# Alexander-H-Liu/End-to-end-ASR-Pytorch

Hardware: AMD Instinct MI355X
Metric: audio frames/sec training (LAS+CTC, LibriSpeech 80-mel) (higher is better)
Workload: dtype f32; 1 GPU; cfg3: {"B": 32, "T": 1600, "D": 80, "V": 5000, "L": 64}; global_batch=32, parallelism=dp1

## Files before the change

end-to-end-asr-pytorch_amd/_lib.py:

```python
import ctypes
import os

_HERE = os.path.dirname(os.path.abspath(__file__))
LIB_PATH = os.path.join(_HERE, "csrc", "libasrk.so")

c_int, c_i64, c_f32, c_vp, c_sz = (ctypes.c_int, ctypes.c_int64, ctypes.c_float, ctypes.c_void_p,
                                   ctypes.c_size_t)
c_f64 = ctypes.c_double

SIGNATURES = {
    "asrk_version": (c_int, []),
    "asrk_strerror": (ctypes.c_char_p, [c_int]),
    "asrk_init": (c_int, [c_int]),
    "asrk_profile_enable": (None, [c_int]),
    "asrk_profile_families": (None, [ctypes.c_uint]),
    "asrk_profile_reset": (None, []),
    "asrk_profile_get": (c_int, [c_int, ctypes.POINTER(ctypes.c_double), ctypes.POINTER(c_i64)]),
    "asrk_profile_get_work": (c_int, [c_int, ctypes.POINTER(ctypes.c_double)]),
    "asrk_gemm_f32": (c_int, [c_int, c_int, c_int, c_int, c_int, c_f32, c_vp, c_int, c_vp, c_int,
                              c_f32, c_vp, c_int, c_vp, c_vp, c_int, c_int, c_vp, c_sz, c_vp]),
    "asrk_gemm_ws_bytes": (c_sz, [c_int, c_int, c_int, c_int]),
    "asrk_gemm_takes_split": (c_int, [c_int, c_int, c_int, c_int]),
    "asrk_gemm_plan_info": (c_int, [c_int, c_int, c_int, c_int, c_int, c_int, c_int, c_int, c_int, c_f32, c_int, c_int,
                                    c_int, c_vp]),
    "asrk_split_panel_bytes": (ctypes.c_size_t, [c_int, c_int, c_int]),
    "asrk_split_panel_f32": (c_int, [c_vp, c_int, c_int, c_int, c_int, c_vp, c_int, c_vp]),
    "asrk_gemm_panels_f32": (c_int, [c_int, c_int, c_int, c_f32, c_vp, c_int, c_int, c_int, c_int,
                                     c_vp, c_int, c_int, c_int, c_int, c_f32, c_vp, c_int, c_vp, c_vp, c_int, c_vp]),
    "asrk_gemm_panels_splitk_ws_bytes": (c_sz, [c_int, c_int, c_int]),
    "asrk_gemm_panels_splitk_f32": (c_int, [c_int, c_int, c_int, c_f32, c_vp, c_int, c_int, c_int, c_int,
                                            c_vp, c_int, c_int, c_int, c_int, c_f32, c_vp, c_int, c_vp, c_vp, c_int,
                                            c_vp, c_sz, c_int, c_vp]),
    "asrk_copy3d_f32": (c_int, [c_vp, c_vp, c_int, c_int, c_int, c_i64, c_i64, c_i64, c_i64, c_int,
                                c_vp]),
    "asrk_colsum_f32": (c_int, [c_vp, c_int, c_int, c_int, c_vp, c_int, c_vp]),
    "asrk_tanh_fwd_f32": (c_int, [c_vp, c_vp, c_i64, c_vp]),
    "asrk_tanh_bwd_f32": (c_int, [c_vp, c_vp, c_vp, c_i64, c_vp]),
    "asrk_log_softmax_fwd_f32": (c_int, [c_vp, c_vp, c_int, c_int, c_int, c_vp]),
    "asrk_log_softmax_bwd_f32": (c_int, [c_vp, c_vp, c_vp, c_int, c_int, c_int, c_vp]),
    "asrk_cross_entropy_fwd_f32": (c_int, [c_vp, c_int, c_int, c_int, c_vp, c_int, c_vp, c_vp, c_vp]),
    "asrk_cross_entropy_bwd_f32": (c_int, [c_vp, c_int, c_int, c_int, c_vp, c_int, c_vp, c_vp, c_vp,
                                           c_vp]),
    "asrk_cross_entropy_ls_fwd_f32": (c_int, [c_vp, c_int, c_int, c_int, c_vp, c_int, c_vp, c_vp, c_vp, c_vp]),
    "asrk_cross_entropy_ls_bwd_f32": (c_int, [c_vp, c_int, c_int, c_int, c_vp, c_int, c_f32, c_vp, c_vp, c_vp,
                                              c_vp]),
    "asrk_ctc_prefix_score_f32": (c_int, [c_vp, c_vp, c_vp, c_vp, c_vp, c_vp, c_vp, c_int, c_int, c_int,
                                          c_int, c_int, c_int, c_f32, c_vp]),
# ... 221 lines not shown
```

end-to-end-asr-pytorch_amd/csrc/gemm_split.hip:

```cpp
#include "common.h"
#include "knobs.h"
#include <algorithm>
#include <climits>

extern "C" int asrk_cu_count_(void);

namespace {

typedef __bf16 bf16x8 __attribute__((ext_vector_type(8)));

constexpr int PIECE = 1024;

struct SplitGemmArgs {
    const unsigned char *Ap, *Bp;
    float *C;
    const float *bias, *bias2;
    int M, N, ldc;
    int KC;
    size_t rb_stride_a, rb_stride_b;
    int nk;
    int tiles_m, tiles_n;
    float alpha, beta;
    int slices, ldw;
    float *ws;
};

__device__ __forceinline__ void split8(const float (&v)[8], u32x4 (&w)[3]) {
    unsigned h[3][8];
#pragma unroll
    for (int e = 0; e < 8; ++e) {
        const float a = v[e];
        const __bf16 b0 = (__bf16)a;
        const float r1 = a - (float)b0;
        const __bf16 b1 = (__bf16)r1;
        const float r2 = r1 - (float)b1;
        const __bf16 b2 = (__bf16)r2;
        h[0][e] = __builtin_bit_cast(unsigned short, b0);
        h[1][e] = __builtin_bit_cast(unsigned short, b1);
        h[2][e] = __builtin_bit_cast(unsigned short, b2);
// ... 109 lines not shown
    const int kt0 = SK ? (int)((long)slice * p.nk / p.slices) : 0;
    const int nk = SK ? (int)((long)(slice + 1) * p.nk / p.slices) - kt0 : p.nk;
    const int q8 = ntiles >> 3, r8 = ntiles & 7, xcd = bid & 7, loc = bid >> 3;
    const int tile = (xcd < r8 ? xcd * (q8 + 1) : r8 * (q8 + 1) + (xcd - r8) * q8) + loc;
    constexpr int BAND = 8;
    const int band = tile / (BAND * p.tiles_m);
    const int band_w = min(BAND, p.tiles_n - band * BAND);
    const int in_band = tile - band * BAND * p.tiles_m;
    const int tm = in_band / band_w, tn = band * BAND + in_band % band_w;

    const bool loader = !SPEC || wave >= NCW, worker = !SPEC || wave < NCW;
    const int wr = worker ? wave >> 1 : 0, wc = wave & 1;
    const int ltm = tm, ltn = tn;
    const int r0 = (SPEC ? wave - NCW : wave) * RPD;
    const unsigned char *gsrc[RPD];
#pragma unroll
    for (int q = 0; q < RPD; ++q) {
        const int r = r0 + q;
        gsrc[q] = (r < WM ? p.Ap + (size_t)(ltm * WM + r) * p.rb_stride_a
                          : p.Bp + (size_t)(ltn * 2 + r - WM) * p.rb_stride_b);
        if (SK) gsrc[q] += (size_t)kt0 * REGION;
    }
    const unsigned voff = lane * 16;
    unsigned char *ldst = lds + r0 * REGION;
    static_assert((NC * NPL) % 4 == 0, "a region is issued as runs of four pieces");
    auto issue = [&](int kt, int stage) {
        unsigned char *l = ldst + stage * STAGE;
#pragma unroll
        for (int q = 0; q < RPD; ++q) {
            const unsigned char *g = gsrc[q] + (size_t)kt * REGION;
#pragma unroll
            for (int j = 0; j < NC * NPL; j += 4) glds16_run<4>(g + j * PIECE, voff, l + q * REGION + j * PIECE);
        }
    };

    f32x16 acc[2][2];
#pragma unroll
    for (int i = 0; i < 2; ++i)
#pragma unroll
        for (int j = 0; j < 2; ++j)
#pragma unroll
            for (int r = 0; r < 16; ++r) acc[i][j][r] = 0.f;

    const int frag_off = ((lane >> 5) * NPL) * PIECE + (lane & 31) * 16;
    const unsigned char *abase = lds + wr * REGION + frag_off;
// ... 184 lines not shown
    const int wave = __builtin_amdgcn_readfirstlane(tid >> 6);
    const int ntiles = p.tiles_m * p.tiles_n, bid = blockIdx.x;
    const int q8 = ntiles >> 3, r8 = ntiles & 7, xcd = bid & 7, loc = bid >> 3;
    const int tile = (xcd < r8 ? xcd * (q8 + 1) : r8 * (q8 + 1) + (xcd - r8) * q8) + loc;
    const int band = tile / (BAND * p.tiles_m);
    const int band_w = min(BAND, p.tiles_n - band * BAND);
    const int in_band = tile - band * BAND * p.tiles_m;
    const int tm = in_band / band_w, tn = band * BAND + in_band % band_w;
    const int nk = p.nk;

    if (wave >= 4) {
        const int d = wave - 4, first = d * LPT;
        constexpr int NRUN = LPT / 3;
        static_assert(NRUN * 3 == LPT, "runs of three pieces");
        const unsigned char *run_g[NRUN];
#pragma unroll
        for (int k = 0; k < NRUN; ++k) {
            const int idx = first + 3 * k, r = idx / (NC * NPL), j = idx - r * (NC * NPL);
            run_g[k] = (r < 2 ? p.Ap + (size_t)(tm * 2 + r) * p.rb_stride_a
                              : p.Bp + (size_t)min(tn * 4 + r - 2, rb_b - 1) * p.rb_stride_b) + j * PIECE;
        }
        const unsigned voff = lane * 16;
        unsigned char *ldst = lds + first * PIECE;
        auto issue = [&](int kt, int stage) {
            unsigned char *l = ldst + stage * STAGE;
            const size_t gk = (size_t)kt * REGION;
#pragma unroll
            for (int k = 0; k < NRUN; ++k) glds16_run<3>(run_g[k] + gk, voff, l + 3 * k * PIECE);
        };
#pragma unroll
        for (int s = 0; s < NST; ++s)
            if (s < nk) issue(s, s);
        {
            const int later = min(NST - 2, nk - 2);
            if (later >= 2) wait_vm<2 * LPT>();
            else if (later == 1) wait_vm<LPT>();
            else wait_vm<0>();
        }
        __builtin_amdgcn_s_barrier();
        int stage = 0;
        for (int kt = 0; kt < nk; ++kt) {
            const int later = min(NST - 2, nk - 2 - kt);
            if (later >= 2) wait_vm<2 * LPT>();
// ... 165 lines not shown
    const int slice = SK ? blockIdx.x / ntiles : 0, bid = SK ? blockIdx.x - slice * ntiles : blockIdx.x;
    const int kt0 = SK ? (int)((long)slice * p.nk / p.slices) : 0;
    const int nk = SK ? (int)((long)(slice + 1) * p.nk / p.slices) - kt0 : p.nk;
    const int q8 = ntiles >> 3, r8 = ntiles & 7, xcd = bid & 7, loc = bid >> 3;
    const int tile = (xcd < r8 ? xcd * (q8 + 1) : r8 * (q8 + 1) + (xcd - r8) * q8) + loc;
    constexpr int BAND = 8;
    const int band = tile / (BAND * p.tiles_m);
    const int band_w = min(BAND, p.tiles_n - band * BAND);
    const int in_band = tile - band * BAND * p.tiles_m;
    const int tm = in_band / band_w, tn = band * BAND + in_band % band_w;

    const bool worker = wave < 4;
    const int wr = worker ? wave >> 1 : 0, wc = wave & 1;
    const int r0 = worker ? 0 : wave - 4;
    const unsigned char *gsrc = (r0 < 2 ? p.Ap + (size_t)(tm * 2 + r0) * p.rb_stride_a
                                        : p.Bp + (size_t)(tn * 2 + r0 - 2) * p.rb_stride_b) + (size_t)kt0 * REGION;
    const unsigned voff = lane * 16;
    unsigned char *ldst = lds + r0 * REGION;
    auto issue = [&](int kt, int stage) {
        const unsigned char *g = gsrc + (size_t)kt * REGION;
        unsigned char *l = ldst + stage * STAGE;
#pragma unroll
        for (int j = 0; j < LPT; j += 4) glds16_run<4>(g + j * PIECE, voff, l + j * PIECE);
    };

    f32x4 acc[4][4];
#pragma unroll
    for (int i = 0; i < 4; ++i)
#pragma unroll
        for (int j = 0; j < 4; ++j)
#pragma unroll
            for (int r = 0; r < 4; ++r) acc[i][j][r] = 0.f;
    const int frag_off = ((lane >> 4) * NPL) * PIECE + (lane & 15) * 16;
    const unsigned char *abase = lds + wr * REGION + frag_off;
    const unsigned char *bbase = lds + (2 + wc) * REGION + frag_off;
// ... 114 lines not shown
    static_assert(LPT * NDW == NRG * NC * NPL && NRUN * 3 == LPT, "36 pieces per stage, runs of three");
    const int tid = threadIdx.x, lane = tid & 63;
    const int wave = __builtin_amdgcn_readfirstlane(tid >> 6);
    const int ntiles = p.tiles_m * p.tiles_n, bid = blockIdx.x;
    const int q8 = ntiles >> 3, r8 = ntiles & 7, xcd = bid & 7, loc = bid >> 3;
    const int tile = (xcd < r8 ? xcd * (q8 + 1) : r8 * (q8 + 1) + (xcd - r8) * q8) + loc;
    const int band = tile / (BAND * p.tiles_m);
    const int band_w = min(BAND, p.tiles_n - band * BAND);
    const int in_band = tile - band * BAND * p.tiles_m;
    const int tm = in_band / band_w, tn = band * BAND + in_band % band_w;
    const int ns = p.nk >> 1;

    const bool worker = wave < 4;
    const int first = (worker ? 0 : wave - 4) * LPT;
    const unsigned char *run_g[NRUN];
#pragma unroll
    for (int k = 0; k < NRUN; ++k) {
        const int idx = first + 3 * k, r = idx / (NC * NPL), j = idx - r * (NC * NPL);
        run_g[k] = (r < 2 ? p.Ap + (size_t)(tm * 2 + r) * p.rb_stride_a
                          : p.Bp + (size_t)min(tn * 4 + r - 2, rb_b - 1) * p.rb_stride_b) + j * PIECE;
    }
    const unsigned voff = lane * 16;
    unsigned char *ldst = lds + first * PIECE;
    auto issue_pair = [&](int s, int slot) {
#pragma unroll
        for (int h = 0; h < 2; ++h) {
            unsigned char *l = ldst + slot * PAIR + h * STAGE;
            const size_t gk = (size_t)(2 * s + h) * REGION;
#pragma unroll
            for (int k = 0; k < NRUN; ++k) glds16_run<3>(run_g[k] + gk, voff, l + 3 * k * PIECE);
        }
    };

    const int wr = worker ? wave >> 1 : 0, wc = wave & 1;
    f32x4 acc0[4][4], acc1[4][4];
#pragma unroll
    for (int i = 0; i < 4; ++i)
#pragma unroll
        for (int j = 0; j < 4; ++j)
#pragma unroll
            for (int r = 0; r < 4; ++r) acc0[i][j][r] = acc1[i][j][r] = 0.f;
    const int frag_off = (lane >> 5) * STAGE + (((lane >> 4) & 1) * NPL) * PIECE + (lane & 15) * 16;
    const unsigned char *abase = lds + wr * REGION + frag_off;
    const unsigned char *bbase = lds + (2 + wc * 2) * REGION + frag_off;
    bf16x8 fa0[2][4], fa1[4], fa2[4], fb0[4], fb1[4], fb2[4];
// ... 161 lines not shown
        else hipLaunchKernelGGL((split_panel_kernel<false>), grid, dim3(256), 0, s, src, ld, rows, K, dstp, g.KC, g.rb, g.rb_stride);
    }
    asrk_prof_end_(PROF_SPLIT, s);
    ASRK_LAUNCH_CHECK();
    return ASRK_OK;
}

int auto_slices(int M, int N, int nk) {
    if (N >= 512) return 1;
    const int ncu = asrk_cu_count_() > 0 ? asrk_cu_count_() : 256;
    const long tiles = (long)asrk_div_up(M, 128) * asrk_div_up(N, 128);
    const long want = (ncu + tiles - 1) / tiles;
    return (int)std::max(1L, std::min(want, (long)(nk / 64)));
}

int run_panel_gemm(int M, int N, int nk, float alpha, const unsigned char *Ap, size_t stride_a,
                   const unsigned char *Bp, size_t stride_b, float beta, float *C, int ldc, const float *bias,
                   const float *bias2, hipStream_t s, int slices = 1, float *ws = nullptr) {
    const AsrkKnobs &kn = asrk_knobs_();
    SplitGemmArgs a;
    a.Ap = Ap; a.Bp = Bp; a.C = C; a.bias = bias; a.bias2 = bias2;
    a.M = M; a.N = N; a.ldc = ldc; a.KC = 0; a.nk = nk; a.rb_stride_a = stride_a; a.rb_stride_b = stride_b;
    a.tiles_m = asrk_div_up(M, 128); a.tiles_n = asrk_div_up(N, 128);
    a.alpha = alpha; a.beta = beta;
    a.slices = std::min(slices, nk); a.ldw = (N + 3) & ~3; a.ws = ws;
    const bool m16 = kn.is_set(kn.split_mfma) ? kn.split_mfma == 16 : nk >= SPLIT_MFMA16_MIN_NK;
    const bool m16_sk = kn.is_set(kn.split_mfma) && kn.split_mfma == 16;
    const bool m16_128 = m16, m16_w256 = m16;
    if (a.slices > 1) return m16_sk ? launch_split_gemm_m16<true>(a, s) : launch_split_gemm<4, 3, true, 2, true>(a, s);
    const int w256 = kn.get(kn.split_w256, 1);
    if (w256 && N >= 512) {
        const int tm = asrk_div_up(M, 128), tn = asrk_div_up(N, 256);
        const int ncu = asrk_cu_count_() > 0 ? asrk_cu_count_() : 256;
        if (w256 == 2 || (long)tm * tn >= 2L * ncu) {
            SplitGemmArgs b = a;
// ... 61 lines not shown
                                    void *stream) {
    if (!src || !panel || rows <= 0 || K <= 0 || ld < (trans ? rows : K) || flags != 0) return ASRK_EINVAL;
    if ((reinterpret_cast<uintptr_t>(panel) & 15) != 0) return ASRK_EINVAL;
    asrk_prof_begin_(PROF_GEMM, (hipStream_t)stream);
    const int rc = run_split(src, ld, rows, K, trans != 0, reinterpret_cast<unsigned char *>(panel),
                             panel_geom(rows, K, true), (hipStream_t)stream);
    asrk_prof_end_(PROF_GEMM, (hipStream_t)stream);
    return rc;
}

namespace {
struct PanelRange {
    const unsigned char *Ap, *Bp;
    size_t stride_a, stride_b;
    int nk;
};
int panel_range(int M, int N, int K, const void *A_panel, int a_rows, int a_K, int a_row0, int a_k0,
                const void *B_panel, int b_rows, int b_K, int b_row0, int b_k0, const float *C, int ldc, int flags,
                PanelRange &r) {
    if (M <= 0 || N <= 0 || K <= 0 || !A_panel || !B_panel || !C || ldc < N || flags != 0) return ASRK_EINVAL;
    if (a_row0 < 0 || b_row0 < 0 || a_k0 < 0 || b_k0 < 0 || a_row0 % 128 || b_row0 % 128 || a_k0 % 8 || b_k0 % 8)
        return ASRK_EINVAL;
    if (a_row0 + M > a_rows || b_row0 + N > b_rows || a_k0 + K > a_K || b_k0 + K > b_K) return ASRK_EINVAL;
    if (K % 32 != 0 && a_k0 + K != a_K && b_k0 + K != b_K) return ASRK_ESHAPE;
    const PanelGeom ga = panel_geom(a_rows, a_K, true), gb = panel_geom(b_rows, b_K, true);
    r.nk = asrk_div_up(K, 32);
    if (a_k0 / 8 + r.nk * SPLIT_NC > ga.KC || b_k0 / 8 + r.nk * SPLIT_NC > gb.KC) return ASRK_ESHAPE;
    const unsigned char *A0 = reinterpret_cast<const unsigned char *>(A_panel);
    const unsigned char *B0 = reinterpret_cast<const unsigned char *>(B_panel);
    r.Ap = A0 + (size_t)(a_row0 / 64) * ga.rb_stride + (size_t)(a_k0 / 8) * NPL * PIECE;
    r.Bp = B0 + (size_t)(b_row0 / 64) * gb.rb_stride + (size_t)(b_k0 / 8) * NPL * PIECE;
    r.stride_a = ga.rb_stride; r.stride_b = gb.rb_stride;
    return ASRK_OK;
}
}
// ... 28 lines not shown
    if (splitk < 0 || !ws || (reinterpret_cast<uintptr_t>(ws) & 15) != 0) return ASRK_EINVAL;
    PanelRange r;
    const int rc0 = panel_range(M, N, K, A_panel, a_rows, a_K, a_row0, a_k0, B_panel, b_rows, b_K, b_row0, b_k0, C, ldc,
                                flags, r);
    if (rc0 != ASRK_OK) return rc0;
    const int slices = splitk > 0 ? splitk : auto_slices(M, N, r.nk);
    if (ws_bytes < asrk_gemm_panels_splitk_ws_bytes(M, N, slices)) return ASRK_EWORKSPACE;
    hipStream_t s = (hipStream_t)stream;
    asrk_prof_work_(PROF_GEMM, 2.0 * (double)M * (double)N * (double)K);
    asrk_prof_begin_(PROF_GEMM, s);
    const int rc = run_panel_gemm(M, N, r.nk, alpha, r.Ap, r.stride_a, r.Bp, r.stride_b, beta, C, ldc, bias, bias2, s,
                                  slices, reinterpret_cast<float *>(ws));
    asrk_prof_end_(PROF_GEMM, s);
    return rc;
}
```

end-to-end-asr-pytorch_amd/ops.py:

```python
import collections
import contextlib
import ctypes

import numpy as np
import torch
from torch.autograd import Function

from . import _lib

_ws_cache = {}


def _L():
    return _lib.load()


def _require_gpu(t):
    if not t.is_cuda:
        raise _lib.AsrkError("asrk ops need tensors on the MI355X (got %s); the product path has no "
                             "CPU fallback" % t.device)


def _p(t):
    return ctypes.c_void_p(t.data_ptr()) if t is not None else ctypes.c_void_p(0)
# ... 149 lines not shown


def join_deferred():
    for dev, ev in list(_defer["pending"].items()):
        torch.cuda.current_stream(dev).wait_event(ev)
    _defer["pending"].clear()


def deferred_stream(device):
    dev = torch.device(device)
    if dev.index is None:
        dev = torch.device(dev.type, torch.cuda.current_device())
    return _defer["side"].get(dev) if dev in _defer["pending"] else None


def _end_of_backward():
    _defer["cb_armed"] = False
    join_deferred()
    rel, _defer["release"] = _defer["release"], []
    for pnl in rel:
        pnl.release()


def _can_defer(*weights):
    return _defer["enabled"] and all(w is None or (w.is_leaf and w.grad is None) for w in weights)


_BG_FORCED = _os.environ.get("ASRK_SIDE_BG")
_BG_HINT = int(_BG_FORCED) if _BG_FORCED is not None else 0


_gemm_phase_hooks = []
# ... 53 lines not shown
        if self.hint:
            _gemm_state["lds_hint"] = self.hint
        return self

    def keep(self, *outs):
        for t in outs:
            if t is not None:
                t.record_stream(self.main)

    def __exit__(self, *exc):
        _gemm_state["lds_hint"] = self.prev_hint
        self.ctx.__exit__(*exc)
        done = torch.cuda.Event()
        done.record(self.side)
        _defer["pending"][self.device] = done
        if not _defer["cb_armed"]:
            try:
                torch.autograd.Variable._execution_engine.queue_callback(_end_of_backward)
                _defer["cb_armed"] = True
            except RuntimeError:
                join_deferred()
        return False


_grad_dest = {"fn": None}


def set_grad_destination(fn):
    _grad_dest["fn"] = fn


def grad_out(weight, shape, device):
    fn = _grad_dest["fn"]
    if fn is not None and weight is not None:
        t = fn(weight, tuple(shape))
        if t is not None:
# ... 34 lines not shown
        avail = src.untyped_storage().nbytes() // src.element_size() - src.storage_offset()
        if ld < (rows if trans else K) or avail < need:
            raise _lib.AsrkError("split panel: source too small for {}x{} (trans={}) with ld {}".format(
                rows, K, trans, ld))
        self.rows, self.K = rows, K
        self.flags = 0
        self.buf = torch.empty((L.asrk_split_panel_bytes(rows, K, self.flags),), dtype=torch.uint8,
                               device=src.device)
        _lib.check(L.asrk_split_panel_f32(_p(src), ld, rows, K, int(trans), _p(self.buf), self.flags, _stream()),
                   "split_panel")


import weakref as _weakref
_REC_PANELS = _os.environ.get("ASRK_REC_PANELS", "1") != "0"
_REC_SKIP_DG = True
_panel_pool = {"free": {}, "bytes": 0, "tick": 0, "seen": {}, "stats": {"hit": 0, "miss": 0, "skipped": 0, "evicted": 0}}
_panel_state = {"hint": False, "handover": None,
                "stats": {"emitted": 0, "consumed": 0, "dg": 0, "dgt": 0, "no_dg": 0, "dw_ih_splitk": 0}}


class _BlankPanel:
    __slots__ = ("buf", "rows", "K", "flags", "key")

    @staticmethod
    def take(rows, K, device):
        key = (device.index, torch.cuda.current_stream(device).cuda_stream, rows, K)
        free = _panel_pool["free"].get(key)
        if free:
            e = free.pop()
            _panel_pool["bytes"] -= e[0].numel()
            _panel_pool["stats"]["hit"] += 1
            return _BlankPanel(rows, K, key, e[0])
        seen = _panel_pool["seen"]
# ... 26 lines not shown
    _panel_state["hint"] = bool(flag)


def _take_handover(x):
    h, _panel_state["handover"] = _panel_state["handover"], None
    if h is None:
        return None
    ref, version, panel = h
    if ref() is x and x._version == version and panel.rows == x.shape[0] * x.shape[1] and panel.K == x.shape[2]:
        return panel
    panel.release()
    return None


def gemm_panels(M, N, K, A, a_row0, a_k0, B, b_row0, b_k0, C, ldc, alpha=1.0, beta=0.0, bias=None, bias2=None,
                splitk=None):
    _require_gpu(C)
    avail = C.untyped_storage().nbytes() // C.element_size() - C.storage_offset()
    if ldc < N or avail < (M - 1) * ldc + N:
        raise _lib.AsrkError("gemm_panels: C too small for {}x{} with ld {}".format(M, N, ldc))
    if A.flags != B.flags:
        raise _lib.AsrkError("gemm_panels: the two panels were built in different layouts")
    L = _L()
    if splitk is None:
        _lib.check(L.asrk_gemm_panels_f32(M, N, K, alpha, _p(A.buf), A.rows, A.K, a_row0, a_k0, _p(B.buf), B.rows,
                                          B.K, b_row0, b_k0, beta, _p(C), ldc, _p(bias), _p(bias2), A.flags,
                                          _stream()), "gemm_panels")
        return
    nws = int(L.asrk_gemm_panels_splitk_ws_bytes(M, N, splitk))
    ws = torch.empty((nws,), dtype=torch.uint8, device=C.device)
    _lib.check(L.asrk_gemm_panels_splitk_f32(M, N, K, alpha, _p(A.buf), A.rows, A.K, a_row0, a_k0, _p(B.buf), B.rows,
                                             B.K, b_row0, b_k0, beta, _p(C), ldc, _p(bias), _p(bias2), splitk, _p(ws),
                                             nws, A.flags, _stream()), "gemm_panels")


def zeros(shape, device):
    t = torch.empty(shape, dtype=torch.float32, device=device)
    if t.numel():
# ... 273 lines not shown
    x = _Exchange(L, T, B, H, ndir, 1, dev)
    db_all = torch.empty((ndir, 4 * H), dtype=torch.float32, device=dev) if has_bias else None
    yield x, db_all
    x.done()
    if has_bias and not _db_in_kernel(has_bias, B):
        colsum(G, T * B, ndir * 4 * H, ndir * 4 * H, db_all)
    _gemm_phase_begins()


STREAM = "STREAM"
SIDE_ALL = "SIDE_ALL"
SIDE_REVERSE_SHARED = "SIDE_REVERSE_SHARED"
SIDE_REVERSE = "SIDE_REVERSE"
IH_PANELS, IH_SPLITK, IH_F32 = "panels", "panels_splitk", "f32"
LstmBwdPlan = collections.namedtuple("LstmBwdPlan", "pG pGT db_in_kernel skip_dg rows_ih dw_ih_route dw_hh_panels "
                                                    "schedule defer_release")


def lstm_bwd_plan(T, B, Din, H, ndir, has_bias, needs_dx, stacked, can_defer, to_scratch, beside_bptt, bf_bwd, share_env,
                  skip_dg_switch, takes_split, take_panel):
    M = T * B
    pG = pGT = None
    if bf_bwd and needs_dx and stacked and takes_split(M, Din, 8 * H):
        pG = take_panel(M, 8 * H)
    share0 = share_env and T > 1 and H % 128 == 0 and B % 8 == 0 and takes_split(4 * H, H, (T - 1) * B)
    if bf_bwd and share0 and B % 16 == 0 and not beside_bptt:
        pGT = take_panel(ndir * 4 * H, M)
    rows_ih = 8 * H if stacked and (needs_dx or not can_defer) and to_scratch else 4 * H
    wide_ih = Din % 4 == 0 and takes_split(rows_ih, Din, M)
    narrow_ih = pGT is not None and Din % 4 == 0 and not wide_ih
    if narrow_ih and stacked and to_scratch:
        rows_ih = 8 * H
    db_in_kernel = _db_in_kernel(has_bias, B)
    skip_dg = bool(skip_dg_switch and pGT is not None and Din % 4 == 0 and (not needs_dx or pG is not None)
                   and (db_in_kernel or not has_bias))
    if not (can_defer and (beside_bptt or not needs_dx)):
        schedule = STREAM
    elif needs_dx or ndir == 1:
        schedule = SIDE_ALL
    elif pGT is None:
        schedule = SIDE_REVERSE
    elif Din % 4 == 0:
        schedule = STREAM
    else:
        schedule = SIDE_REVERSE_SHARED
    panels = bool(share0) and schedule != SIDE_REVERSE
    route = IH_SPLITK if narrow_ih else IH_PANELS if panels and wide_ih else IH_F32
    return LstmBwdPlan(pG, pGT, db_in_kernel, skip_dg, rows_ih, route, panels, schedule, schedule == SIDE_REVERSE_SHARED)


class LSTMLayerFn(Function):

    @staticmethod
    def forward(ctx, x, w_ih_f, w_hh_f, b_ih_f, b_hh_f, w_ih_r, w_hh_r, b_ih_r, b_hh_r, pyr_rate=1,
                pyr_style=None):
        _require_gpu(x)
        L = _L()
        xc = _f32c(x)
        T, B, Din = xc.shape
        H = w_hh_f.shape[1]
        ndir = 2 if w_ih_r is not None else 1
        dev = x.device
        M = T * B
        G = torch.empty((M, ndir * 4 * H), dtype=torch.float32, device=dev)
        w_ih_f, w_hh_f = _f32c(w_ih_f), _f32c(w_hh_f)
        w_stack = None
        if ndir == 2:
            w_ih_r, w_hh_r = _f32c(w_ih_r), _f32c(w_hh_r)
        if ndir == 2 and H >= 768 and _os.environ.get("ASRK_STACK_DIRS", "1") != "0":
            if (w_ih_f.untyped_storage().data_ptr() == w_ih_r.untyped_storage().data_ptr()
                    and w_ih_r.storage_offset() == w_ih_f.storage_offset() + 4 * H * Din):
                w_stack = w_ih_f.as_strided((8 * H, Din), (Din, 1))
            else:
                w_stack = torch.empty((8 * H, Din), dtype=torch.float32, device=dev)
                copy_flat(w_stack[:4 * H], w_ih_f)
                copy_flat(w_stack[4 * H:], w_ih_r)
            if b_ih_f is not None:
                b1 = torch.empty((2, 8 * H), dtype=torch.float32, device=dev)
# ... 34 lines not shown
            _lib.check(L.asrk_lstm_rec_fwd_pyr_panel_f32(_p(G), _p(w_hh_f), _p(w_hh_r), _p(Y), _p(C), T, B, H, ndir,
                                                         _p(xc_.buf), xc_.prefilled, _p(ws), _p(Y2), mode, rate,
                                                         _p(out_panel.buf), xc_.flags, _stream()), "lstm_rec_fwd")
        else:
            _lib.check(L.asrk_lstm_rec_fwd_pyr_f32(_p(G), _p(w_hh_f), _p(w_hh_r), _p(Y), _p(C), T, B, H, ndir,
                                                   _p(xc_.buf), xc_.prefilled, _p(ws), _p(Y2), mode, rate,
                                                   xc_.flags, _stream()), "lstm_rec_fwd")
        xc_.done()
        ctx.pyr = (mode, max(1, pyr_rate))
        ctx.dims = (T, B, Din, H, ndir)
        ctx.has_bias = b_ih_f is not None
        ctx.bias_refs = (b_ih_f, b_hh_f, b_ih_r, b_hh_r)
        ctx.save_for_backward(xc, w_ih_f, w_hh_f, w_ih_r, w_hh_r, G, C, Y, w_stack)
        ctx.consumed = False
        out = Y2 if mode else Y.view(T, B, ndir * H)
        if _panel_state["handover"] is not None:
            _panel_state["handover"][2].release()
            _panel_state["handover"] = None
        if out_panel is not None:
            _panel_state["handover"] = (_weakref.ref(out), out._version, out_panel)
        return out

    @staticmethod
    def backward(ctx, dY):
        L = _L()
        xc, w_ih_f, w_hh_f, w_ih_r, w_hh_r, G, C, Y, w_stack = ctx.saved_tensors
        if ctx.consumed:
            raise RuntimeError("LSTMLayerFn: backward twice (the gate buffer is reused in place)")
        ctx.consumed = True
        T, B, Din, H, ndir = ctx.dims
        dev = dY.device
        M = T * B
        ldg, ldy = ndir * 4 * H, ndir * H
        mode, rate = ctx.pyr
        dYc = _f32c(dY)
        ws = lstm_workspace(dev)
        needs_dx = ctx.needs_input_grad[0]
        w_ih, w_hh = (w_ih_f, w_ih_r), (w_hh_f, w_hh_r)
        with _bptt_launch(L, T, B, H, ndir, ctx.has_bias, G, dev) as (xc_, db_all):
            plan = lstm_bwd_plan(T, B, Din, H, ndir, ctx.has_bias, needs_dx, w_stack is not None,
                                 _can_defer(w_ih_f, w_hh_f, w_ih_r, w_hh_r, *ctx.bias_refs),
                                 not grad_has_destination(*w_ih[:ndir]), _defer_beside_bptt(),
                                 bool(_REC_PANELS and L.asrk_lstm_plan_is_bf(T, B, H, ndir, 1, rec_flags(1))),
                                 _os.environ.get("ASRK_SHARE_PANELS", "1") != "0", _REC_SKIP_DG, gemm_takes_split,
                                 lambda rows, K: _BlankPanel.take(rows, K, dev))
            pG, pGT = plan.pG, plan.pGT
            stats = _panel_state["stats"]
            stats["dg"] += pG is not None
            stats["dgt"] += pGT is not None
            stats["no_dg"] += plan.skip_dg
            stats["dw_ih_splitk"] += (plan.dw_ih_route == IH_SPLITK) * (1 if plan.rows_ih == 8 * H else ndir)
            db = db_all if plan.db_in_kernel else None
            if pG is not None or pGT is not None:
                _lib.check(L.asrk_lstm_rec_bwd_pyr_panel_f32(_p(G), _p(w_hh_f), _p(w_hh_r), _p(C), _p(dYc), T, B, H,
                                                             ndir, _p(xc_.buf), xc_.prefilled, _p(ws), _p(db), mode, rate,
                                                             _p(pG.buf if pG is not None else None),
                                                             _p(pGT.buf if pGT is not None else None),
                                                             xc_.flags | (ASRK_REC_BWD_NO_DG if plan.skip_dg else 0),
                                                             _stream()), "lstm_rec_bwd")
            else:
                _lib.check(L.asrk_lstm_rec_bwd_pyr_f32(_p(G), _p(w_hh_f), _p(w_hh_r), _p(C), _p(dYc), T, B, H,
                                                       ndir, _p(xc_.buf), xc_.prefilled, _p(ws), _p(db), mode, rate,
                                                       xc_.flags, _stream()), "lstm_rec_bwd")
        dG = G
        f32 = dict(dtype=torch.float32, device=dev)
        dx = None
# ... 7 lines not shown
            elif w_stack is not None:
                gemm(0, 0, M, Din, 8 * H, dG, ldg, w_stack, Din, dx, Din)
            else:
                gemm(0, 0, M, Din, 4 * H, dG, ldg, w_ih_f, Din, dx, Din)
                if ndir == 2:
                    gemm(0, 0, M, Din, 4 * H, dG[:, 4 * H:], ldg, w_ih_r, Din, dx, Din, beta=1.0)
            dx = dx.view(T, B, Din)
        panels = {} if pGT is None else {"dGT": pGT}
        dw_ih_stack = []

        def panel(name, src, ld, rows):
            if name not in panels:
                panels[name] = SplitPanel(src, ld, rows, M, True)
            return panels[name]

        def dg_gemm(Mo, No, Ko, m0, k0, pB, b_row0, b_k0, out, ldo, splitk=None):
            gemm_panels(Mo, No, Ko, panel("dGT", dG, ldg, ldg), m0, k0, pB, b_row0, b_k0, out, ldo, splitk=splitk)

        def dw_ih_of(d):
            stacked = plan.rows_ih == 8 * H
            if not (stacked and dw_ih_stack):
                out = torch.empty((8 * H, Din), **f32) if stacked else grad_out(w_ih[d], (4 * H, Din), dev)
                m0 = 0 if stacked else d * 4 * H
                if plan.dw_ih_route == IH_F32:
                    gemm(1, 0, plan.rows_ih, Din, M, dG[:, m0:], ldg, xc, Din, out, Din)
                else:
                    dg_gemm(plan.rows_ih, Din, M, m0, 0, panel("XT", xc, Din, Din), 0, 0, out, Din,
                            0 if plan.dw_ih_route == IH_SPLITK else None)
                if not stacked:
                    return out
                dw_ih_stack.append(out)
            return dw_ih_stack[0][d * 4 * H:(d + 1) * 4 * H]

        def dw_hh_of(d):
            if T <= 1:
                return zeros((4 * H, H), dev)
            out, Mh = grad_out(w_hh[d], (4 * H, H), dev), (T - 1) * B
            if plan.dw_hh_panels:
                dg_gemm(4 * H, H, Mh, d * 4 * H, B if d == 0 else 0, panel("YT", Y, ldy, ldy), d * H, 0 if d == 0 else B,
                        out, H)
            elif d == 0:
                gemm(1, 0, 4 * H, H, Mh, dG[B:], ldg, Y, ldy, out, H)
            else:
                gemm(1, 0, 4 * H, H, Mh, dG[:, 4 * H:], ldg, Y[B:, H:], ldy, out, H)
            return out

        def param_grads(d):
            if plan.dw_hh_panels:
                dw_hh = dw_hh_of(d)
                dw_ih = dw_ih_of(d)
            else:
                dw_ih = dw_ih_of(d)
                dw_hh = dw_hh_of(d)
# ... 5 lines not shown

        if plan.schedule == STREAM:
            grads = [param_grads(d) for d in range(ndir)]
        elif plan.schedule == SIDE_ALL:
            with _SideStream(dev, (dG, xc, Y, db_all)) as side:
                grads = [param_grads(d) for d in range(ndir)]
                side.keep(*[t for g in grads for t in g])
        else:
            inputs = (dG, xc, Y, db_all)
            if plan.schedule == SIDE_REVERSE_SHARED:
                inputs += (pGT.buf, panel("YT", Y, ldy, ldy).buf)
            with _SideStream(dev, inputs, background=False) as side:
                g1 = param_grads(1)
                side.keep(*g1)
            grads = [param_grads(0), g1]
        if pGT is not None:
            if plan.defer_release or _defer["pending"]:
                _defer["release"].append(pGT)
            else:
                pGT.release()
        if ndir == 1:
            grads.append((None, None, None, None))
        return (dx,) + grads[0] + grads[1] + (None, None)


class Copy3dFn(Function):

    @staticmethod
    def forward(ctx, src, out_shape, n0, n1, n2, ss0, ss1, ds0, ds1):
        _require_gpu(src)
# ... 807 lines not shown
```

include/asrk.h:

```cpp
#ifndef ASRK_H
#define ASRK_H

#include <stddef.h>
#include <stdint.h>

#ifdef __cplusplus
extern "C" {
#endif

#define ASRK_OK 0
#define ASRK_EINVAL (-1)
#define ASRK_ESHAPE (-2)
#define ASRK_EWORKSPACE (-3)
#define ASRK_EDEVICE (-4)
#define ASRK_ETIMEOUT (-5)

int asrk_version(void);
const char *asrk_strerror(int rc);
int asrk_init(int device);

void asrk_profile_enable(int on);
void asrk_profile_families(unsigned mask);
void asrk_profile_reset(void);
int asrk_profile_get(int id, double *total_ms, int64_t *launches);
// ... 27 lines not shown
#define ASRK_GEMM_PLAN_INFO_LEN 16
int asrk_gemm_plan_info(int transA, int transB, int M, int N, int K, int lda, int ldb, int ldc, int align,
                        float beta, int splitk, int flags, int ncu, int *info);

size_t asrk_split_panel_bytes(int rows, int K, int flags);
int asrk_split_panel_f32(const float *src, int ld, int rows, int K, int trans, void *panel, int flags, void *stream);
int asrk_gemm_panels_f32(int M, int N, int K, float alpha, const void *A_panel, int a_rows, int a_K,
                         int a_row0, int a_k0, const void *B_panel, int b_rows, int b_K, int b_row0, int b_k0,
                         float beta, float *C, int ldc, const float *bias, const float *bias2, int flags,
                         void *stream);
size_t asrk_gemm_panels_splitk_ws_bytes(int M, int N, int splitk);
int asrk_gemm_panels_splitk_f32(int M, int N, int K, float alpha, const void *A_panel, int a_rows, int a_K,
                                int a_row0, int a_k0, const void *B_panel, int b_rows, int b_K, int b_row0, int b_k0,
                                float beta, float *C, int ldc, const float *bias, const float *bias2, int splitk,
                                void *ws, size_t ws_bytes, int flags, void *stream);

int asrk_copy3d_f32(const float *src, float *dst, int n0, int n1, int n2,
                    int64_t s_stride0, int64_t s_stride1, int64_t d_stride0, int64_t d_stride1,
                    int accumulate, void *stream);

int asrk_colsum_f32(const float *X, int M, int N, int ldx, float *out, int accumulate,
                    void *stream);

int asrk_tanh_fwd_f32(const float *x, float *y, int64_t n, void *stream);
int asrk_tanh_bwd_f32(const float *y, const float *dy, float *dx, int64_t n, void *stream);

int asrk_log_softmax_fwd_f32(const float *x, float *y, int rows, int cols, int ld,
                             void *stream);
int asrk_log_softmax_bwd_f32(const float *y, const float *dy, float *dx, int rows, int cols,
                             int ld, void *stream);
// ... 416 lines not shown
```

Baseline: 556,700 frames/s.

## Reuse the upper LSTM layer's transposed-input panel as the lower layer's YT panel

```diff
diff --git a/end-to-end-asr-pytorch_amd/_lib.py b/end-to-end-asr-pytorch_amd/_lib.py
--- a/end-to-end-asr-pytorch_amd/_lib.py
+++ b/end-to-end-asr-pytorch_amd/_lib.py
@@ -31,6 +31,9 @@
     "asrk_gemm_panels_splitk_f32": (c_int, [c_int, c_int, c_int, c_f32, c_vp, c_int, c_int, c_int, c_int,
                                             c_vp, c_int, c_int, c_int, c_int, c_f32, c_vp, c_int, c_vp, c_vp, c_int,
                                             c_vp, c_sz, c_int, c_vp]),
+    "asrk_gemm_panels_phase_f32": (c_int, [c_int, c_int, c_int, c_f32, c_vp, c_int, c_int, c_int, c_int,
+                                           c_vp, c_int, c_int, c_int, c_int, c_int, c_int, c_f32, c_vp, c_int, c_vp,
+                                           c_vp, c_int, c_vp, c_sz, c_int, c_vp]),
     "asrk_copy3d_f32": (c_int, [c_vp, c_vp, c_int, c_int, c_int, c_i64, c_i64, c_i64, c_i64, c_int,
                                 c_vp]),
     "asrk_colsum_f32": (c_int, [c_vp, c_int, c_int, c_int, c_vp, c_int, c_vp]),
diff --git a/end-to-end-asr-pytorch_amd/csrc/gemm_split.hip b/end-to-end-asr-pytorch_amd/csrc/gemm_split.hip
--- a/end-to-end-asr-pytorch_amd/csrc/gemm_split.hip
+++ b/end-to-end-asr-pytorch_amd/csrc/gemm_split.hip
@@ -23,6 +23,23 @@
     float alpha, beta;
     int slices, ldw;
     float *ws;
+    int b_j0, b_sh, b_mask;
+    size_t b_pstride;
+};
+
+struct KtileMap {
+    int j0, sh, mask;
+    size_t pstride;
+    __device__ __forceinline__ void set(const SplitGemmArgs &p, bool is_b, int kt0) {
+        j0 = kt0 + (is_b ? p.b_j0 : 0);
+        sh = is_b ? p.b_sh : 0;
+        mask = is_b ? p.b_mask : 0;
+        pstride = is_b ? p.b_pstride : 0;
+    }
+    __device__ __forceinline__ size_t at(int kt, int TILE) const {
+        const int j = j0 + kt;
+        return (size_t)(j >> sh) * TILE + (size_t)(j & mask) * pstride;
+    }
 };
 
 __device__ __forceinline__ void split8(const float (&v)[8], u32x4 (&w)[3]) {
@@ -162,12 +179,13 @@
     const int ltm = tm, ltn = tn;
     const int r0 = (SPEC ? wave - NCW : wave) * RPD;
     const unsigned char *gsrc[RPD];
+    KtileMap kmap[RPD];
 #pragma unroll
     for (int q = 0; q < RPD; ++q) {
         const int r = r0 + q;
         gsrc[q] = (r < WM ? p.Ap + (size_t)(ltm * WM + r) * p.rb_stride_a
                           : p.Bp + (size_t)(ltn * 2 + r - WM) * p.rb_stride_b);
-        if (SK) gsrc[q] += (size_t)kt0 * REGION;
+        kmap[q].set(p, r >= WM, kt0);
     }
     const unsigned voff = lane * 16;
     unsigned char *ldst = lds + r0 * REGION;
@@ -176,7 +194,8 @@
         unsigned char *l = ldst + stage * STAGE;
 #pragma unroll
         for (int q = 0; q < RPD; ++q) {
-            const unsigned char *g = gsrc[q] + (size_t)kt * REGION;
+            static_assert(NC == 4, "a region is one 32-k tile of the panel");
+            const unsigned char *g = gsrc[q] + kmap[q].at(kt, REGION);
 #pragma unroll
             for (int j = 0; j < NC * NPL; j += 4) glds16_run<4>(g + j * PIECE, voff, l + q * REGION + j * PIECE);
         }
@@ -391,19 +410,22 @@
         constexpr int NRUN = LPT / 3;
         static_assert(NRUN * 3 == LPT, "runs of three pieces");
         const unsigned char *run_g[NRUN];
+        KtileMap kmap[NRUN];
 #pragma unroll
         for (int k = 0; k < NRUN; ++k) {
             const int idx = first + 3 * k, r = idx / (NC * NPL), j = idx - r * (NC * NPL);
             run_g[k] = (r < 2 ? p.Ap + (size_t)(tm * 2 + r) * p.rb_stride_a
                               : p.Bp + (size_t)min(tn * 4 + r - 2, rb_b - 1) * p.rb_stride_b) + j * PIECE;
+            kmap[k].set(p, r >= 2, 0);
         }
         const unsigned voff = lane * 16;
         unsigned char *ldst = lds + first * PIECE;
         auto issue = [&](int kt, int stage) {
             unsigned char *l = ldst + stage * STAGE;
-            const size_t gk = (size_t)kt * REGION;
-#pragma unroll
-            for (int k = 0; k < NRUN; ++k) glds16_run<3>(run_g[k] + gk, voff, l + 3 * k * PIECE);
+            const size_t half = (size_t)(kt & 1) * REGION;
+#pragma unroll
+            for (int k = 0; k < NRUN; ++k)
+                glds16_run<3>(run_g[k] + kmap[k].at(kt >> 1, 2 * REGION) + half, voff, l + 3 * k * PIECE);
         };
 #pragma unroll
         for (int s = 0; s < NST; ++s)
@@ -599,11 +621,13 @@
     const int wr = worker ? wave >> 1 : 0, wc = wave & 1;
     const int r0 = worker ? 0 : wave - 4;
     const unsigned char *gsrc = (r0 < 2 ? p.Ap + (size_t)(tm * 2 + r0) * p.rb_stride_a
-                                        : p.Bp + (size_t)(tn * 2 + r0 - 2) * p.rb_stride_b) + (size_t)kt0 * REGION;
+                                        : p.Bp + (size_t)(tn * 2 + r0 - 2) * p.rb_stride_b);
+    KtileMap kmap;
+    kmap.set(p, r0 >= 2, kt0);
     const unsigned voff = lane * 16;
     unsigned char *ldst = lds + r0 * REGION;
     auto issue = [&](int kt, int stage) {
-        const unsigned char *g = gsrc + (size_t)kt * REGION;
+        const unsigned char *g = gsrc + kmap.at(kt, REGION);
         unsigned char *l = ldst + stage * STAGE;
 #pragma unroll
         for (int j = 0; j < LPT; j += 4) glds16_run<4>(g + j * PIECE, voff, l + j * PIECE);
@@ -748,11 +772,13 @@
     const bool worker = wave < 4;
     const int first = (worker ? 0 : wave - 4) * LPT;
     const unsigned char *run_g[NRUN];
+    KtileMap kmap[NRUN];
 #pragma unroll
     for (int k = 0; k < NRUN; ++k) {
         const int idx = first + 3 * k, r = idx / (NC * NPL), j = idx - r * (NC * NPL);
         run_g[k] = (r < 2 ? p.Ap + (size_t)(tm * 2 + r) * p.rb_stride_a
                           : p.Bp + (size_t)min(tn * 4 + r - 2, rb_b - 1) * p.rb_stride_b) + j * PIECE;
+        kmap[k].set(p, r >= 2, 0);
     }
     const unsigned voff = lane * 16;
     unsigned char *ldst = lds + first * PIECE;
@@ -760,9 +786,9 @@
 #pragma unroll
         for (int h = 0; h < 2; ++h) {
             unsigned char *l = ldst + slot * PAIR + h * STAGE;
-            const size_t gk = (size_t)(2 * s + h) * REGION;
-#pragma unroll
-            for (int k = 0; k < NRUN; ++k) glds16_run<3>(run_g[k] + gk, voff, l + 3 * k * PIECE);
+#pragma unroll
+            for (int k = 0; k < NRUN; ++k)
+                glds16_run<3>(run_g[k] + kmap[k].at(s, 2 * REGION) + (size_t)h * REGION, voff, l + 3 * k * PIECE);
         }
     };
 
@@ -954,11 +980,17 @@
     return (int)std::max(1L, std::min(want, (long)(nk / 64)));
 }
 
+struct BPhase {
+    int j0 = 0, sh = 0, mask = 0;
+    size_t pstride = 0;
+};
+
 int run_panel_gemm(int M, int N, int nk, float alpha, const unsigned char *Ap, size_t stride_a,
                    const unsigned char *Bp, size_t stride_b, float beta, float *C, int ldc, const float *bias,
-                   const float *bias2, hipStream_t s, int slices = 1, float *ws = nullptr) {
+                   const float *bias2, hipStream_t s, int slices = 1, float *ws = nullptr, const BPhase &ph = BPhase()) {
     const AsrkKnobs &kn = asrk_knobs_();
     SplitGemmArgs a;
+    a.b_j0 = ph.j0; a.b_sh = ph.sh; a.b_mask = ph.mask; a.b_pstride = ph.pstride;
     a.Ap = Ap; a.Bp = Bp; a.C = C; a.bias = bias; a.bias2 = bias2;
     a.M = M; a.N = N; a.ldc = ldc; a.KC = 0; a.nk = nk; a.rb_stride_a = stride_a; a.rb_stride_b = stride_b;
     a.tiles_m = asrk_div_up(M, 128); a.tiles_n = asrk_div_up(N, 128);
@@ -1050,11 +1082,40 @@
     const unsigned char *Ap, *Bp;
     size_t stride_a, stride_b;
     int nk;
+    BPhase ph;
 };
+int panel_range_phases(int N, int K, int b_rows, int b_K, int b_row0, int b_k0, int phases, int phase_rows,
+                       const PanelGeom &gb, const void *B_panel, PanelRange &r) {
+    if (phases < 2 || phases > 64 || (phases & (phases - 1)) || phase_rows <= 0 || phase_rows % 128) return ASRK_EINVAL;
+    if (b_k0 % 32 || K % 32 || b_K % 32) return ASRK_ESHAPE;
+    if (b_row0 + N > phase_rows || (long)phases * phase_rows > b_rows) return ASRK_EINVAL;
+    if ((long)b_k0 + K > (long)phases * b_K) return ASRK_EINVAL;
+    int sh = 0;
+    while ((1 << sh) < phases) ++sh;
+    r.ph.j0 = b_k0 / 32; r.ph.sh = sh; r.ph.mask = phases - 1;
+    r.ph.pstride = (size_t)(phase_rows / 64) * gb.rb_stride;
+    r.Bp = reinterpret_cast<const unsigned char *>(B_panel) + (size_t)(b_row0 / 64) * gb.rb_stride;
+    return ASRK_OK;
+}
 int panel_range(int M, int N, int K, const void *A_panel, int a_rows, int a_K, int a_row0, int a_k0,
                 const void *B_panel, int b_rows, int b_K, int b_row0, int b_k0, const float *C, int ldc, int flags,
-                PanelRange &r) {
+                PanelRange &r, int b_phases = 1, int b_phase_rows = 0) {
     if (M <= 0 || N <= 0 || K <= 0 || !A_panel || !B_panel || !C || ldc < N || flags != 0) return ASRK_EINVAL;
+    if (b_phases < 1 || b_phase_rows < 0) return ASRK_EINVAL;
+    if (b_phases > 1) {
+        if (a_row0 < 0 || b_row0 < 0 || a_k0 < 0 || b_k0 < 0 || a_row0 % 128 || b_row0 % 128 || a_k0 % 8)
+            return ASRK_EINVAL;
+        if (a_row0 + M > a_rows || a_k0 + K > a_K) return ASRK_EINVAL;
+        const PanelGeom ga = panel_geom(a_rows, a_K, true), gb = panel_geom(b_rows, b_K, true);
+        r.nk = K / 32;
+        if (a_k0 / 8 + r.nk * SPLIT_NC > ga.KC) return ASRK_ESHAPE;
+        const int rc = panel_range_phases(N, K, b_rows, b_K, b_row0, b_k0, b_phases, b_phase_rows, gb, B_panel, r);
+        if (rc != ASRK_OK) return rc;
+        r.Ap = reinterpret_cast<const unsigned char *>(A_panel) + (size_t)(a_row0 / 64) * ga.rb_stride +
+               (size_t)(a_k0 / 8) * NPL * PIECE;
+        r.stride_a = ga.rb_stride; r.stride_b = gb.rb_stride;
+        return ASRK_OK;
+    }
     if (a_row0 < 0 || b_row0 < 0 || a_k0 < 0 || b_k0 < 0 || a_row0 % 128 || b_row0 % 128 || a_k0 % 8 || b_k0 % 8)
         return ASRK_EINVAL;
     if (a_row0 + M > a_rows || b_row0 + N > b_rows || a_k0 + K > a_K || b_k0 + K > b_K) return ASRK_EINVAL;
@@ -1113,3 +1174,25 @@
     asrk_prof_end_(PROF_GEMM, s);
     return rc;
 }
+
+extern "C" int asrk_gemm_panels_phase_f32(int M, int N, int K, float alpha, const void *A_panel, int a_rows, int a_K,
+                                          int a_row0, int a_k0, const void *B_panel, int b_rows, int b_K, int b_row0,
+                                          int b_k0, int b_phases, int b_phase_rows, float beta, float *C, int ldc,
+                                          const float *bias, const float *bias2, int splitk, void *ws,
+                                          size_t ws_bytes, int flags, void *stream) {
+    if (splitk < 0) return ASRK_EINVAL;
+    if (splitk != 1 && (!ws || (reinterpret_cast<uintptr_t>(ws) & 15) != 0)) return ASRK_EINVAL;
+    PanelRange r;
+    const int rc0 = panel_range(M, N, K, A_panel, a_rows, a_K, a_row0, a_k0, B_panel, b_rows, b_K, b_row0, b_k0, C, ldc,
+                                flags, r, b_phases, b_phase_rows);
+    if (rc0 != ASRK_OK) return rc0;
+    const int slices = splitk > 0 ? splitk : auto_slices(M, N, r.nk);
+    if (splitk != 1 && ws_bytes < asrk_gemm_panels_splitk_ws_bytes(M, N, slices)) return ASRK_EWORKSPACE;
+    hipStream_t s = (hipStream_t)stream;
+    asrk_prof_work_(PROF_GEMM, 2.0 * (double)M * (double)N * (double)K);
+    asrk_prof_begin_(PROF_GEMM, s);
+    const int rc = run_panel_gemm(M, N, r.nk, alpha, r.Ap, r.stride_a, r.Bp, r.stride_b, beta, C, ldc, bias, bias2, s,
+                                  slices, reinterpret_cast<float *>(ws), r.ph);
+    asrk_prof_end_(PROF_GEMM, s);
+    return rc;
+}
diff --git a/end-to-end-asr-pytorch_amd/ops.py b/end-to-end-asr-pytorch_amd/ops.py
--- a/end-to-end-asr-pytorch_amd/ops.py
+++ b/end-to-end-asr-pytorch_amd/ops.py
@@ -187,8 +187,19 @@
     return _defer["side"].get(dev) if dev in _defer["pending"] else None
 
 
+def _arm_end_of_backward():
+    if not _defer["cb_armed"]:
+        try:
+            torch.autograd.Variable._execution_engine.queue_callback(_end_of_backward)
+            _defer["cb_armed"] = True
+        except RuntimeError:
+            return False
+    return True
+
+
 def _end_of_backward():
     _defer["cb_armed"] = False
+    _panel_state["xt"] = None
     join_deferred()
     rel, _defer["release"] = _defer["release"], []
     for pnl in rel:
@@ -272,12 +283,8 @@
         done = torch.cuda.Event()
         done.record(self.side)
         _defer["pending"][self.device] = done
-        if not _defer["cb_armed"]:
-            try:
-                torch.autograd.Variable._execution_engine.queue_callback(_end_of_backward)
-                _defer["cb_armed"] = True
-            except RuntimeError:
-                join_deferred()
+        if not _arm_end_of_backward():
+            join_deferred()
         return False
 
 
@@ -342,9 +349,10 @@
 import weakref as _weakref
 _REC_PANELS = _os.environ.get("ASRK_REC_PANELS", "1") != "0"
 _REC_SKIP_DG = True
+_SHARE_YT = True
 _panel_pool = {"free": {}, "bytes": 0, "tick": 0, "seen": {}, "stats": {"hit": 0, "miss": 0, "skipped": 0, "evicted": 0}}
-_panel_state = {"hint": False, "handover": None,
-                "stats": {"emitted": 0, "consumed": 0, "dg": 0, "dgt": 0, "no_dg": 0, "dw_ih_splitk": 0}}
+_panel_state = {"hint": False, "handover": None, "last_out": None, "xt": None,
+                "stats": {"emitted": 0, "consumed": 0, "dg": 0, "dgt": 0, "no_dg": 0, "dw_ih_splitk": 0, "yt_shared": 0}}
 
 
 class _BlankPanel:
@@ -401,7 +409,7 @@
 
 
 def gemm_panels(M, N, K, A, a_row0, a_k0, B, b_row0, b_k0, C, ldc, alpha=1.0, beta=0.0, bias=None, bias2=None,
-                splitk=None):
+                splitk=None, b_phases=1, b_phase_rows=0):
     _require_gpu(C)
     avail = C.untyped_storage().nbytes() // C.element_size() - C.storage_offset()
     if ldc < N or avail < (M - 1) * ldc + N:
@@ -409,6 +417,15 @@
     if A.flags != B.flags:
         raise _lib.AsrkError("gemm_panels: the two panels were built in different layouts")
     L = _L()
+    if b_phases != 1:
+        one = splitk is None or splitk == 1
+        nws = 0 if one else int(L.asrk_gemm_panels_splitk_ws_bytes(M, N, splitk))
+        ws = torch.empty((nws,), dtype=torch.uint8, device=C.device) if nws else None
+        _lib.check(L.asrk_gemm_panels_phase_f32(M, N, K, alpha, _p(A.buf), A.rows, A.K, a_row0, a_k0, _p(B.buf), B.rows,
+                                                B.K, b_row0, b_k0, b_phases, b_phase_rows, beta, _p(C), ldc, _p(bias),
+                                                _p(bias2), 1 if one else splitk, _p(ws), nws, A.flags, _stream()),
+                   "gemm_panels")
+        return
     if splitk is None:
         _lib.check(L.asrk_gemm_panels_f32(M, N, K, alpha, _p(A.buf), A.rows, A.K, a_row0, a_k0, _p(B.buf), B.rows,
                                           B.K, b_row0, b_k0, beta, _p(C), ldc, _p(bias), _p(bias2), A.flags,
@@ -712,11 +729,12 @@
 SIDE_REVERSE = "SIDE_REVERSE"
 IH_PANELS, IH_SPLITK, IH_F32 = "panels", "panels_splitk", "f32"
 LstmBwdPlan = collections.namedtuple("LstmBwdPlan", "pG pGT db_in_kernel skip_dg rows_ih dw_ih_route dw_hh_panels "
-                                                    "schedule defer_release")
+                                                    "schedule defer_release yt_share")
+YtShare = collections.namedtuple("YtShare", "phases phase_rows row0 a_k0 b_k0")
 
 
 def lstm_bwd_plan(T, B, Din, H, ndir, has_bias, needs_dx, stacked, can_defer, to_scratch, beside_bptt, bf_bwd, share_env,
-                  skip_dg_switch, takes_split, take_panel):
+                  skip_dg_switch, takes_split, take_panel, above_xt=None):
     M = T * B
     pG = pGT = None
     if bf_bwd and needs_dx and stacked and takes_split(M, Din, 8 * H):
@@ -744,7 +762,13 @@
         schedule = SIDE_REVERSE_SHARED
     panels = bool(share0) and schedule != SIDE_REVERSE
     route = IH_SPLITK if narrow_ih else IH_PANELS if panels and wide_ih else IH_F32
-    return LstmBwdPlan(pG, pGT, db_in_kernel, skip_dg, rows_ih, route, panels, schedule, schedule == SIDE_REVERSE_SHARED)
+    yt_share = None
+    if (above_xt is not None and panels and B == 32 and above_xt[0] >= 2 and above_xt[0] & (above_xt[0] - 1) == 0
+            and T % above_xt[0] == 0 and (ndir * H) % 128 == 0 and above_xt[1] == schedule
+            and schedule in (STREAM, SIDE_ALL)):
+        yt_share = YtShare(above_xt[0], ndir * H, tuple(d * H for d in range(ndir)), (B, 0)[:ndir], (0, B)[:ndir])
+    return LstmBwdPlan(pG, pGT, db_in_kernel, skip_dg, rows_ih, route, panels, schedule, schedule == SIDE_REVERSE_SHARED,
+                       yt_share)
 
 
 class LSTMLayerFn(Function):
@@ -760,6 +784,8 @@
         ndir = 2 if w_ih_r is not None else 1
         dev = x.device
         M = T * B
+        below, _panel_state["last_out"] = _panel_state["last_out"], None
+        ctx.x_token = below[2] if (below is not None and x is xc and below[0]() is x and x._version == below[1]) else None
         G = torch.empty((M, ndir * 4 * H), dtype=torch.float32, device=dev)
         w_ih_f, w_hh_f = _f32c(w_ih_f), _f32c(w_hh_f)
         w_stack = None
@@ -824,6 +850,9 @@
         ctx.save_for_backward(xc, w_ih_f, w_hh_f, w_ih_r, w_hh_r, G, C, Y, w_stack)
         ctx.consumed = False
         out = Y2 if mode else Y.view(T, B, ndir * H)
+        ctx.y2_token = object() if mode == 1 else None
+        if mode == 1:
+            _panel_state["last_out"] = (_weakref.ref(out), out._version, ctx.y2_token)
         if _panel_state["handover"] is not None:
             _panel_state["handover"][2].release()
             _panel_state["handover"] = None
@@ -847,19 +876,27 @@
         ws = lstm_workspace(dev)
         needs_dx = ctx.needs_input_grad[0]
         w_ih, w_hh = (w_ih_f, w_ih_r), (w_hh_f, w_hh_r)
+        main_stream = torch.cuda.current_stream(dev).cuda_stream
+        offer, _panel_state["xt"] = _panel_state["xt"], None
+        above_xt = xt_panel = None
+        if (offer is not None and ctx.y2_token is not None and offer["token"] is ctx.y2_token and _REC_PANELS and _SHARE_YT
+                and offer["stream"] == main_stream and offer["shape"] == (T // rate, B, rate * ldy)):
+            above_xt, xt_panel = (rate, offer["schedule"]), offer["panel"]
+        del offer
         with _bptt_launch(L, T, B, H, ndir, ctx.has_bias, G, dev) as (xc_, db_all):
             plan = lstm_bwd_plan(T, B, Din, H, ndir, ctx.has_bias, needs_dx, w_stack is not None,
                                  _can_defer(w_ih_f, w_hh_f, w_ih_r, w_hh_r, *ctx.bias_refs),
                                  not grad_has_destination(*w_ih[:ndir]), _defer_beside_bptt(),
                                  bool(_REC_PANELS and L.asrk_lstm_plan_is_bf(T, B, H, ndir, 1, rec_flags(1))),
                                  _os.environ.get("ASRK_SHARE_PANELS", "1") != "0", _REC_SKIP_DG, gemm_takes_split,
-                                 lambda rows, K: _BlankPanel.take(rows, K, dev))
+                                 lambda rows, K: _BlankPanel.take(rows, K, dev), above_xt)
             pG, pGT = plan.pG, plan.pGT
             stats = _panel_state["stats"]
             stats["dg"] += pG is not None
             stats["dgt"] += pGT is not None
             stats["no_dg"] += plan.skip_dg
             stats["dw_ih_splitk"] += (plan.dw_ih_route == IH_SPLITK) * (1 if plan.rows_ih == 8 * H else ndir)
+            stats["yt_shared"] += plan.yt_share is not None
             db = db_all if plan.db_in_kernel else None
             if pG is not None or pGT is not None:
                 _lib.check(L.asrk_lstm_rec_bwd_pyr_panel_f32(_p(G), _p(w_hh_f), _p(w_hh_r), _p(C), _p(dYc), T, B, H,
@@ -897,8 +934,9 @@
                 panels[name] = SplitPanel(src, ld, rows, M, True)
             return panels[name]
 
-        def dg_gemm(Mo, No, Ko, m0, k0, pB, b_row0, b_k0, out, ldo, splitk=None):
-            gemm_panels(Mo, No, Ko, panel("dGT", dG, ldg, ldg), m0, k0, pB, b_row0, b_k0, out, ldo, splitk=splitk)
+        def dg_gemm(Mo, No, Ko, m0, k0, pB, b_row0, b_k0, out, ldo, splitk=None, **phase_map):
+            gemm_panels(Mo, No, Ko, panel("dGT", dG, ldg, ldg), m0, k0, pB, b_row0, b_k0, out, ldo, splitk=splitk,
+                        **phase_map)
 
         def dw_ih_of(d):
             stacked = plan.rows_ih == 8 * H
@@ -919,7 +957,11 @@
             if T <= 1:
                 return zeros((4 * H, H), dev)
             out, Mh = grad_out(w_hh[d], (4 * H, H), dev), (T - 1) * B
-            if plan.dw_hh_panels:
+            ys = plan.yt_share
+            if ys is not None:
+                dg_gemm(4 * H, H, Mh, d * 4 * H, ys.a_k0[d], xt_panel, ys.row0[d], ys.b_k0[d], out, H,
+                        b_phases=ys.phases, b_phase_rows=ys.phase_rows)
+            elif plan.dw_hh_panels:
                 dg_gemm(4 * H, H, Mh, d * 4 * H, B if d == 0 else 0, panel("YT", Y, ldy, ldy), d * H, 0 if d == 0 else B,
                         out, H)
             elif d == 0:
@@ -955,6 +997,10 @@
                 g1 = param_grads(1)
                 side.keep(*g1)
             grads = [param_grads(0), g1]
+        if ("XT" in panels and ctx.x_token is not None and _REC_PANELS and _SHARE_YT and
+                plan.schedule in (STREAM, SIDE_ALL) and _arm_end_of_backward()):
+            _panel_state["xt"] = dict(panel=panels["XT"], schedule=plan.schedule, stream=main_stream, token=ctx.x_token,
+                                      shape=tuple(xc.shape))
         if pGT is not None:
             if plan.defer_release or _defer["pending"]:
                 _defer["release"].append(pGT)
diff --git a/include/asrk.h b/include/asrk.h
--- a/include/asrk.h
+++ b/include/asrk.h
@@ -65,6 +65,10 @@
                                 int a_row0, int a_k0, const void *B_panel, int b_rows, int b_K, int b_row0, int b_k0,
                                 float beta, float *C, int ldc, const float *bias, const float *bias2, int splitk,
                                 void *ws, size_t ws_bytes, int flags, void *stream);
+int asrk_gemm_panels_phase_f32(int M, int N, int K, float alpha, const void *A_panel, int a_rows, int a_K,
+                               int a_row0, int a_k0, const void *B_panel, int b_rows, int b_K, int b_row0, int b_k0,
+                               int b_phases, int b_phase_rows, float beta, float *C, int ldc, const float *bias,
+                               const float *bias2, int splitk, void *ws, size_t ws_bytes, int flags, void *stream);
 
 int asrk_copy3d_f32(const float *src, float *dst, int n0, int n1, int n2,
                     int64_t s_stride0, int64_t s_stride1, int64_t d_stride0, int64_t d_stride1,
```

Result: no change. 554,500 frames/s (-0.4%).
